# menmitsu/opticalFlowClustering

Measured on AMD Instinct MI355X. Metric: Mpixels/s dense flow+kmeans @1080p, higher is better.
Workload: dtype f32 storage, f64 accumulation; 1 GPU; BASELINE.json configs[2]: 300-frame 1080p synthetic clip, Farneback flow (0.5,3,15,3,5,1.2,0) + Lloyd k=5 over (u,v), frames sharded over 1 GPU(s); width=1920, height=1080, frames=300, pairs=299, k=5, lloyd_iters=11, flow_batch_pairs=64

## Files before the change

include/ofc.h:

```cpp
#ifndef OFC_H
#define OFC_H
#include <stddef.h>
#include <stdint.h>

#ifdef __cplusplus
extern "C" {
#endif

#define OFC_VERSION 100

enum {
    OFC_OK = 0,
    OFC_EINVAL = -1,
    OFC_ENODEV = -2,
    OFC_EHIP = -3,
    OFC_ENOMEM = -4,
    OFC_ENOTREADY = -5,
    OFC_EUNSUPPORTED = -6,
    OFC_ECOMM = -7
};

enum { OFC_U8 = 0, OFC_F32 = 1, OFC_F64 = 2 };

int ofc_version(void);
// ... 70 lines not shown
int ofc_bench_polyexp(int device, int W, int H, int n_images, int iters, int rows_per_block,
                      float *ms_per_launch);

int ofc_bgr2gray(int device, const uint8_t *bgr, int W, int H, uint8_t *gray);
int ofc_flow_to_bgr(int device, const float *flow, int W, int H, uint8_t *bgr, float *mean_mag);
int ofc_flow_to_bgr_dev(int device, const float *flow_dev, int W, int H, int n_frames,
                        uint8_t *bgr_dev, float *mean_mag_dev);
int ofc_bgr2hsv(int device, const uint8_t *bgr, int64_t npix, uint8_t *hsv);
int ofc_preprocess_rgba(int device, const uint8_t *img3, int64_t npix, int thresh, uint8_t *rgba);
int ofc_grid_cell_means(int device, const uint8_t *bgr, int W, int H, int rows, int cols,
                        uint8_t *mean_bgr, uint8_t *hsv);

int ofc_kmeans_fit(int device, const void *X, int dtype, int64_t N, int d, int k,
                   const double *init, int max_iter, double tol_rel, double *centers,
                   int32_t *labels, double *inertia, int *n_iter);
int ofc_kmeans_predict(int device, const void *X, int dtype, int64_t N, int d, int k,
                       const double *centers, int32_t *labels);
int ofc_kmeans_fit_dev(int device, const void *X_dev, int dtype, int64_t N, int d, int k,
                       const double *init, int max_iter, double tol_rel, double *centers,
                       uint8_t *labels_dev, double *inertia, int *n_iter);
int ofc_kmeans_fit_dev_stats(int device, const void *X_dev, int dtype, int64_t N, int d, int k,
                             const double *init, int max_iter, double tol_rel, const double *colsum,
                             double *centers, uint8_t *labels_dev, double *inertia, int *n_iter);
int ofc_kmeans_fit_dev_field(int device, const void *X_dev, int dtype, int64_t N, int d, int k,
                             const double *init, int max_iter, double tol_rel, const double *colsum,
                             double *centers, uint8_t *labels_dev, double *inertia, int *n_iter,
                             int W, int H, int64_t n_fields);
int64_t ofc_lloyd_field_origin(int64_t tile, int quad, int W);
int ofc_lloyd_field_origins(int64_t tile0, int64_t n_tiles, int W, int64_t *out);
void ofc_lloyd_field_shape(int *tile_w, int *tile_h, int *group_w, int *group_h);
int ofc_lloyd_prune_stats(int device, double *out6);
int ofc_bench_lloyd_sweep(int device, const float *X_dev, int64_t N, int k, const double *centers, const double *mean,
                          int what, int iters, float *ms_per_launch);
int ofc_lloyd_colstats_dev(int device, const void *X_dev, int dtype, int64_t N, int d, const double *mean,
                           int pass, double *out);
int ofc_lloyd_step_dev(int device, const void *X_dev, int dtype, int64_t N, int d, int k, const double *mean,
                       const double *centers_c, uint8_t *labels_dev, int accumulate, double *record);
int ofc_lloyd_inertia_dev(int device, const void *X_dev, int dtype, int64_t N, int d, int k, const double *mean,
                          const double *centers_c, const uint8_t *labels_dev, double *inertia);
int ofc_lloyd_farthest_dev(int device, const void *X_dev, int dtype, int64_t N, int d, int k, const double *mean,
                           const double *centers_c, const uint8_t *labels_dev, const int64_t *excl, int n_excl,
                           double *dist2, int64_t *index, double *x_c, int *label);

int ofc_kmeans_fit_w(int device, const void *X, int dtype, const void *w, int w_dtype, int64_t N, int d, int k,
                     const double *init, int max_iter, double tol_rel, double *centers, int32_t *labels,
                     double *inertia, int *n_iter);
int ofc_kmeans_fit_dev_w(int device, const void *X_dev, int dtype, const void *w_dev, int w_dtype, int64_t N, int d,
                         int k, const double *init, int max_iter, double tol_rel, const double *colsum,
                         double *centers, uint8_t *labels_dev, double *inertia, int *n_iter);
int ofc_kmeans_score(int device, const void *X, int dtype, const void *w, int w_dtype, int64_t N, int d, int k,
                     const double *centers, double *inertia);
int ofc_lloyd_step_dev_w(int device, const void *X_dev, int dtype, const void *w_dev, int w_dtype, int64_t N, int d,
                         int k, const double *mean, const double *centers_c, uint8_t *labels_dev, double *record);
int ofc_lloyd_inertia_dev_w(int device, const void *X_dev, int dtype, const void *w_dev, int w_dtype, int64_t N, int d,
                            int k, const double *mean, const double *centers_c, const uint8_t *labels_dev,
                            double *inertia);
int ofc_lloyd_farthest_dev_w(int device, const void *X_dev, int dtype, const void *w_dev, int w_dtype, int64_t N, int d,
                             int k, const double *mean, const double *centers_c, const uint8_t *labels_dev,
                             const int64_t *excl, int n_excl, double *dist2, int64_t *index, double *x_c, int *label,
                             double *weight);
int ofc_flow_weights_dev(int device, const float *flow_dev, int64_t n, int kind, float thr, float *w_dev);
int ofc_bench_lloyd_sweep_w(int device, const float *X_dev, const void *w_dev, int w_dtype, int64_t N, int k,
                            const double *centers, const double *mean, int iters, float *ms_per_launch);

int ofc_kpp_candidates(int device, const void *X, int dtype, int64_t N, int d, const double *mean,
                       const int64_t *cand, int n_cand, const double *closest, double *out_min, double *pots);
// ... 189 lines not shown
```

opticalflowclustering_amd/_lib.py:

```python
import ctypes as C
import os

import numpy as np

_HERE = os.path.dirname(os.path.abspath(__file__))
LIB_PATH = os.path.join(_HERE, "libofc.so")

OFC_OK, OFC_EINVAL, OFC_ENODEV, OFC_EHIP, OFC_ENOMEM, OFC_ENOTREADY, OFC_EUNSUPPORTED, OFC_ECOMM = \
    0, -1, -2, -3, -4, -5, -6, -7
U8, F32, F64 = 0, 1, 2
UNIQUE_ID_BYTES = 128
KPP_CHUNK = 1024
UV_HIST_SHARE = 2048
UV_HIST_MAX_GRID = 2048
BLOB_TILE_W, BLOB_TILE_H, BLOB_FIELDS = 64, 16, 12
BLOB_LINK_FIELDS, BLOB_NO_MOVE = 3, -0x7fff8000
CONSIST_OK, CONSIST_MISMATCH, CONSIST_LEAVES, CONSIST_INVALID, CONSIST_STATES = 0, 1, 2, 3, 4
CONSIST_SHARE, CONSIST_MAX_DIM = 2048, 16384
CONSIST_ALPHA_MAX, CONSIST_BETA_MAX = 65536, 1 << 62
PHOTO_SHARE, PHOTO_TAU_MAX, PHOTO_KAPPA_MAX, PHOTO_NSTAT = 2048, 65280, 1024, 5
REPAIR_ROUNDS_MAX, REPAIR_NCOUNT, REPAIR_UNFILLED = 254, 3, 255
TRAJ_RAN, TRAJ_UNTRUSTED, TRAJ_LEAVES, TRAJ_INVALID = 0, 1, 2, 3
TRAJ_THREADS, TRAJ_MAX_POINTS = 256, 1 << 28
TRAJ_ONE_LAUNCH_POINTS, TRAJ_DENSE_PAIRS = 1 << 19, 16
# ... 44 lines not shown
    "ofc_flow_push_bgr": ([_vp, _vp, _vp, C.POINTER(_f), _vp], _i),
    "ofc_flow_last_vis_dev": ([_vp, C.POINTER(_vp)], _i),
    "ofc_level_image": ([_i, _vp, _i, _i, C.POINTER(FbParams), _i, _vp, _ip, _ip], _i),
    "ofc_polyexp": ([_i, _vp, _i, _i, _i, _d, _vp], _i),
    "ofc_polyexp_u8": ([_i, _vp, _i, _i, _i, _d, _vp], _i),
    "ofc_update_matrices": ([_i, _vp, _vp, _vp, _i, _i, _vp], _i),
    "ofc_box_solve": ([_i, _vp, _i, _i, _i, _vp], _i),
    "ofc_flow_resize": ([_i, _vp, _i, _i, _i, _i, _f, _vp], _i),
    "ofc_flow_iterate": ([_i, _vp, _vp, _vp, _i, _i, _i, _i, _i, _i, _vp], _i),
    "ofc_flow_launch_geometry": ([_i, _i, _i, _i, _ip], _i),
    "ofc_flow_launch_geometry_bidir": ([_i, _i, _i, _i, _ip], _i),
    "ofc_bench_flow_bidir": ([_i, _i, _i, _i, _i, _i, C.POINTER(_f)], _i),
    "ofc_pyramid_dec": ([_i, _vp, _i, _i, _i, _i, _i, _vp, _vp, _vp, _ip], _i),
    "ofc_pyramid_dec_geometry": ([_i, _i, _i, _ip], _i),
    "ofc_bench_pyramid_dec": ([_i, _i, _i, _i, _i, _i, _i, C.POINTER(_f)], _i),
    "ofc_bench_flow_iters": ([_i, _i, _i, _i, _i, _i, C.POINTER(_f)], _i),
    "ofc_bench_polyexp": ([_i, _i, _i, _i, _i, _i, C.POINTER(_f)], _i),
    "ofc_bgr2gray": ([_i, _vp, _i, _i, _vp], _i),
    "ofc_flow_to_bgr": ([_i, _vp, _i, _i, _vp, C.POINTER(_f)], _i),
    "ofc_flow_to_bgr_dev": ([_i, _vp, _i, _i, _i, _vp, _vp], _i),
    "ofc_bgr2hsv": ([_i, _vp, _i64, _vp], _i),
    "ofc_preprocess_rgba": ([_i, _vp, _i64, _i, _vp], _i),
    "ofc_grid_cell_means": ([_i, _vp, _i, _i, _i, _i, _vp, _vp], _i),
    "ofc_kmeans_fit": ([_i, _vp, _i, _i64, _i, _i, _vp, _i, _d, _vp, _vp, C.POINTER(_d), _ip], _i),
    "ofc_kmeans_predict": ([_i, _vp, _i, _i64, _i, _i, _vp, _vp], _i),
    "ofc_kmeans_fit_dev": ([_i, _vp, _i, _i64, _i, _i, _vp, _i, _d, _vp, _vp, C.POINTER(_d), _ip], _i),
    "ofc_kmeans_fit_dev_stats": ([_i, _vp, _i, _i64, _i, _i, _vp, _i, _d, _vp, _vp, _vp, C.POINTER(_d), _ip], _i),
    "ofc_kmeans_fit_dev_field": ([_i, _vp, _i, _i64, _i, _i, _vp, _i, _d, _vp, _vp, _vp, C.POINTER(_d), _ip, _i, _i, _i64], _i),
    "ofc_lloyd_field_origin": ([_i64, _i, _i], _i64),
    "ofc_lloyd_field_origins": ([_i64, _i64, _i, _vp], _i),
    "ofc_lloyd_field_shape": ([_ip, _ip, _ip, _ip], None),
    "ofc_lloyd_prune_stats": ([_i, _vp], _i),
    "ofc_bench_lloyd_sweep": ([_i, _vp, _i64, _i, _vp, _vp, _i, _i, C.POINTER(_f)], _i),
    "ofc_lloyd_colstats_dev": ([_i, _vp, _i, _i64, _i, _vp, _i, _vp], _i),
    "ofc_lloyd_step_dev": ([_i, _vp, _i, _i64, _i, _i, _vp, _vp, _vp, _i, _vp], _i),
    "ofc_lloyd_inertia_dev": ([_i, _vp, _i, _i64, _i, _i, _vp, _vp, _vp, C.POINTER(_d)], _i),
    "ofc_lloyd_farthest_dev": ([_i, _vp, _i, _i64, _i, _i, _vp, _vp, _vp, _vp, _i, C.POINTER(_d), C.POINTER(_i64), _vp, _ip], _i),
    "ofc_kmeans_fit_w": ([_i, _vp, _i, _vp, _i, _i64, _i, _i, _vp, _i, _d, _vp, _vp, C.POINTER(_d), _ip], _i),
    "ofc_kmeans_fit_dev_w": ([_i, _vp, _i, _vp, _i, _i64, _i, _i, _vp, _i, _d, _vp, _vp, _vp, C.POINTER(_d), _ip], _i),
    "ofc_kmeans_score": ([_i, _vp, _i, _vp, _i, _i64, _i, _i, _vp, C.POINTER(_d)], _i),
    "ofc_lloyd_step_dev_w": ([_i, _vp, _i, _vp, _i, _i64, _i, _i, _vp, _vp, _vp, _vp], _i),
    "ofc_lloyd_inertia_dev_w": ([_i, _vp, _i, _vp, _i, _i64, _i, _i, _vp, _vp, _vp, C.POINTER(_d)], _i),
    "ofc_lloyd_farthest_dev_w": ([_i, _vp, _i, _vp, _i, _i64, _i, _i, _vp, _vp, _vp, _vp, _i, C.POINTER(_d), C.POINTER(_i64), _vp, _ip,
                                  C.POINTER(_d)], _i),
    "ofc_flow_weights_dev": ([_i, _vp, _i64, _i, _f, _vp], _i),
    "ofc_bench_lloyd_sweep_w": ([_i, _vp, _vp, _i, _i64, _i, _vp, _vp, _i, C.POINTER(_f)], _i),
    "ofc_kpp_candidates": ([_i, _vp, _i, _i64, _i, _vp, _vp, _i, _vp, _vp, _vp], _i),
    "ofc_kpp_seed_dev": ([_i, _vp, _i, _i64, _i, _i, _vp, _i64, _vp, _i, _vp, _vp], _i),
    "ofc_kpp_sample_dev": ([_i, _vp, _i64, _vp, _i, _vp], _i),
    "ofc_kpp_seed_dev_w": ([_i, _vp, _i, _vp, _i, _i64, _i, _i, _vp, _d, _vp, _i, _vp, _vp], _i),
    "ofc_kpp_sample_dev_w": ([_i, _vp, _i, _vp, _i64, _vp, _i, _i, _vp, _vp], _i),
    "ofc_kmeans_fit_batched": ([_i, _vp, _vp, _i, _i, _i, _vp, _i, _d, _vp, _vp, _vp, _vp], _i),
    "ofc_grid_kmeans": ([_i, _vp, _i, _i, _i, _i, _i, _vp, _i, _d, _i, _vp, _vp], _i),
    "ofc_grid_kmeans_dev": ([_i, _vp, _i, _i, _i, _i, _i, _i, _vp, _i, _d, _i, _vp, _vp], _i),
    "ofc_dist_unique_id": ([_vp], _i),
    "ofc_dist_init": ([_i, _i, _i, _vp], _i),
    "ofc_dist_allreduce_f64": ([_i, _vp, _i], _i),
    "ofc_dist_init_host": ([_i, _i, _i, _vp, _vp], _i),
    "ofc_dist_loopback": ([_i], _i),
    "ofc_dist_finalize": ([], _i),
    "ofc_stream_create": ([_i, _i, _i, C.POINTER(FbParams), _i, _i, _i, C.POINTER(_vp)], _i),
    "ofc_stream_push_gray": ([_vp, _vp, _ip], _i),
    "ofc_stream_finish": ([_vp, _vp, _i, _ip], _i),
    "ofc_stream_set_model": ([_vp, _i, _vp, _vp, _i], _i),
    "ofc_stream_finish_clusters": ([_vp, _vp, _vp, _vp, _i, _ip], _i),
    "ofc_stream_set_histogram": ([_vp, _i, _f], _i),
# ... 138 lines not shown
```

opticalflowclustering_amd/csrc/lloyd_api.cpp:

```cpp
#include "host_util.h"
#include "lloyd_common.h"

#include <algorithm>
#include <cmath>
#include <cstdlib>
#include <mutex>

namespace ofc {

static int lloyd_grid(int64_t N)
{
    return (int)std::max<int64_t>(1, std::min<int64_t>(cdiv64(N / 4, 256), N >= (200ll << 20) ? 2048 : 1024));
}

static size_t dtype_size(int dtype) { return dtype == OFC_U8 ? 1 : (dtype == OFC_F32 ? 4 : 8); }

struct LloydScratch {
    DevBuf state, partial, tot, tot_local, excl, far, labels;
    DevBuf tile_block;
    DevBuf tile_meta;
    DevBuf kpp_closest, kpp_cs, kpp_ss;
    DevBuf kpp_io;
    double prune_stats[6] = {0, 0, 0, 0, 0, 0};
    LloydStatus *status = nullptr;
// ... 142 lines not shown
    return OFC_OK;
}

static int lloyd_fit_dev(int device, const void *X, int dtype, int64_t N, int d, int k, const double *init,
                         int max_iter, double tol_rel, double *centers, uint8_t *labels_dev,
                         double *inertia, int *n_iter, const double *colsum = nullptr, const void *wdev = nullptr,
                         int w_dtype = OFC_F32, int field_w = 0, int field_h = 0, int64_t n_fields = 0)
{
    OFC_REQUIRE(X && init && centers, "null pointer");
    OFC_REQUIRE(dtype >= OFC_U8 && dtype <= OFC_F64, "bad dtype %d", dtype);
    OFC_REQUIRE(!wdev || w_dtype == OFC_F32 || w_dtype == OFC_F64, "bad weight dtype %d (OFC_F32 or OFC_F64)", w_dtype);
    OFC_REQUIRE(d >= 1 && k >= 1 && max_iter >= 1 && N >= 0, "bad shape");
    if (d > LLOYD_DMAX || k > LLOYD_KMAX) {
        set_error("k=%d, d=%d outside the kernels' range (k <= %d, d <= %d)", k, d, LLOYD_KMAX, LLOYD_DMAX);
        return OFC_EUNSUPPORTED;
    }
    OFC_TRY(ensure_device(device));
    const int kmax = lloyd_kmax(k);
    const int NV = lloyd_record_len(kmax, d);
    LloydScratch &sc = scratch_for(device);
    std::lock_guard<std::mutex> lock(sc.mu);
    OFC_TRY(sc.init());
    hipStream_t s = sc.stream;
    const int nblocks = lloyd_grid(N);
    if (!labels_dev) {
        OFC_TRY(reserve(sc.labels, (size_t)std::max<int64_t>(N, 1)));
        labels_dev = sc.labels.as<uint8_t>();
    }
    LloydState *st = sc.state.as<LloydState>();
    OFC_HIP(hipMemsetAsync(st, 0, sizeof(LloydState), s));
    double *tot = sc.tot.as<double>();

    double hbuf[LLOYD_DMAX + 1], mean_h[LLOYD_DMAX];
    if (colsum) {
        OFC_HIP(hipMemcpyAsync(tot, colsum, sizeof(double) * d, hipMemcpyHostToDevice, s));
    } else {
        OFC_TRY(launch_lloyd_colstats(X, dtype, N, d, st->mean, 0, sc.partial.as<double>(), nblocks, s));
        OFC_TRY(launch_reduce_records(sc.partial.as<double>(), nblocks, d, tot, s));
    }
    double nloc = (double)N;
    OFC_HIP(hipMemcpyAsync(tot + d, &nloc, sizeof(double), hipMemcpyHostToDevice, s));
    OFC_TRY(dist_allreduce_f64(tot, d + 1, DIST_SUM, s));
    OFC_HIP(hipMemcpyAsync(hbuf, tot, sizeof(double) * (d + 1), hipMemcpyDeviceToHost, s));
    OFC_HIP(hipStreamSynchronize(s));
    const double Ng = hbuf[d];
    if (Ng < (double)k) {
        set_error("n_samples=%.0f should be >= n_clusters=%d.", Ng, k);
        return OFC_EINVAL;
    }
    for (int f = 0; f < d; f++) mean_h[f] = hbuf[f] / Ng;
    OFC_HIP(hipMemcpyAsync(st->mean, mean_h, sizeof(double) * d, hipMemcpyHostToDevice, s));

    double c0[LLOYD_KMAX * LLOYD_DMAX];
    for (int j = 0; j < k * d; j++) c0[j] = init[j] - mean_h[j % d];
    OFC_HIP(hipMemcpyAsync(st->centers, c0, sizeof(double) * k * d, hipMemcpyHostToDevice, s));
    const int prune = wdev ? LLOYD_PRUNE_OFF : prune_policy_for(dtype, N, d, k);
    const bool field = prune && field_w > 0 && field_geometry_ok(field_w, field_h, n_fields);
    LloydFieldBufs tb = {};
    if (prune) OFC_TRY(sc.tile_bufs(N, field ? field_w : 0, tb));
    auto tiles_launch = [&](uint8_t *lab, int what, const double *meta) -> int {
        if (field) return launch_lloyd_tiles_field((const float *)X, N, k, st, tb, lab, sc.partial.as<double>(), nblocks, what, meta, s);
        return launch_lloyd_tiles((const float *)X, N, k, st, tb.box, tb.tsum, tb.tsq, lab, sc.partial.as<double>(), nblocks, what,
                                  meta, s);
    };
    for (double &v : sc.prune_stats) v = 0;
    OFC_TRY(launch_lloyd_set_centers(st, k, d, s, prune));
    bool strict = false, labelled = false, stop = false;
    int tiles_next = LLOYD_TILES_FULL;
    const bool trace = getenv("OFC_LLOYD_TRACE") != nullptr;
    int it = 0;
    const int *halt = &st->halt;
    double *tot_local = dist_has_comm() ? sc.tot_local.as<double>() : tot;
    int window = 4;
    while (it < max_iter && !stop) {
        const int nwin = std::min(window, max_iter - it);
        window = std::min(2 * window, LLOYD_WINDOW);
        for (int w = 0; w < nwin; w++) sc.status[w].valid = 0;
// ... 132 lines not shown
    std::lock_guard<std::mutex> lock(sc.mu);
    OFC_TRY(sc.init());
    hipStream_t s = sc.stream;
    const int nblocks = lloyd_grid(N);
    LloydFieldBufs tb = {};
    OFC_TRY(sc.tile_bufs(N, 0, tb));
    OFC_TRY(reserve(sc.labels, (size_t)N));
    LloydState *st = sc.state.as<LloydState>();
    OFC_HIP(hipMemsetAsync(st, 0, sizeof(LloydState), s));
    double c0[LLOYD_KMAX * LLOYD_DMAX];
    for (int j = 0; j < k * 2; j++) c0[j] = centers[j] - mean[j % 2];
    OFC_HIP(hipMemcpyAsync(st->mean, mean, sizeof(double) * 2, hipMemcpyHostToDevice, s));
    OFC_HIP(hipMemcpyAsync(st->centers, c0, sizeof(double) * k * 2, hipMemcpyHostToDevice, s));
    OFC_TRY(launch_lloyd_set_centers(st, k, 2, s, LLOYD_PRUNE_ALWAYS));
    double *partial = sc.partial.as<double>();
    const float *X = X_dev;
    auto launch = [&]() -> int {
        switch (what) {
        case 0: return launch_lloyd_assign(X, OFC_F32, N, 2, k, st, sc.labels.as<uint8_t>(), partial, nblocks, 3, 0, s);
        case 1: case 5: return launch_lloyd_tiles(X, N, k, st, tb.box, tb.tsum, tb.tsq, nullptr, partial, nblocks, LLOYD_WHAT_SWEEP, nullptr, s);
        case 2: return launch_lloyd_tiles(X, N, k, st, tb.box, tb.tsum, tb.tsq, nullptr, partial, nblocks, LLOYD_WHAT_META, nullptr, s);
        case 3: return launch_lloyd_assign(X, OFC_F32, N, 2, k, st, sc.labels.as<uint8_t>(), partial, nblocks, 2, 0, s);
        default: return launch_lloyd_tiles(X, N, k, st, tb.box, tb.tsum, tb.tsq, sc.labels.as<uint8_t>(), partial, nblocks, LLOYD_WHAT_FINAL, nullptr, s);
        }
    };
    if (what == 1 || what == 4 || what == 5) {
        OFC_TRY(launch_lloyd_tiles(X, N, k, st, tb.box, tb.tsum, tb.tsq, nullptr, partial, nblocks, LLOYD_WHAT_META, nullptr, s));
        const int mode = what == 5 ? LLOYD_TILES_FULL : LLOYD_TILES_PRUNED;
        OFC_HIP(hipMemcpyAsync(&st->prune_mode, &mode, sizeof(int), hipMemcpyHostToDevice, s));
    }
    return time_launches(s, iters, launch, ms_per_launch);
}

int ofc_lloyd_prune_stats(int device, double *out6)
{
    OFC_REQUIRE(out6, "null pointer");
    OFC_TRY(ensure_device(device));
    LloydScratch &sc = scratch_for(device);
    std::lock_guard<std::mutex> lock(sc.mu);
    for (int i = 0; i < 6; i++) out6[i] = sc.prune_stats[i];
    return OFC_OK;
}

int ofc_kmeans_fit_dev_stats(int device, const void *X_dev, int dtype, int64_t N, int d, int k, const double *init,
                             int max_iter, double tol_rel, const double *colsum, double *centers, uint8_t *labels_dev,
                             double *inertia, int *n_iter)
{
    return lloyd_fit_dev(device, X_dev, dtype, N, d, k, init, max_iter, tol_rel, centers, labels_dev, inertia, n_iter, colsum);
}

int ofc_kmeans_fit_dev_field(int device, const void *X_dev, int dtype, int64_t N, int d, int k, const double *init,
                             int max_iter, double tol_rel, const double *colsum, double *centers, uint8_t *labels_dev,
                             double *inertia, int *n_iter, int W, int H, int64_t n_fields)
{
    OFC_REQUIRE(dtype == OFC_F32 && d == 2, "a stack of (u,v) fields is float32 with d = 2 (got dtype %d, d = %d)", dtype, d);
    OFC_REQUIRE(W >= 1 && H >= 1 && n_fields >= 1 && N / W / H == n_fields && n_fields * W * H == N,
                "N=%lld is not %lld fields of %d x %d", (long long)N, (long long)n_fields, W, H);
    return lloyd_fit_dev(device, X_dev, dtype, N, d, k, init, max_iter, tol_rel, centers, labels_dev, inertia, n_iter, colsum,
                         nullptr, OFC_F32, W, H, n_fields);
}

int64_t ofc_lloyd_field_origin(int64_t tile, int quad, int W)
{
    if (tile < 0 || quad < 0 || quad > 15 || W < FIELD_GW || W % FIELD_GW) return -1;
    return field_quad_origin(tile, quad, W);
}
// ... 758 lines not shown
```

opticalflowclustering_amd/csrc/lloyd_field.h:

```cpp
#pragma once
#include <cstdint>

#ifndef __host__
#define __host__
#define __device__
#endif

namespace ofc {

#ifndef OFC_FIELD_TW
#define OFC_FIELD_TW 16
#endif
constexpr int FIELD_TW = OFC_FIELD_TW, FIELD_TH = 64 / FIELD_TW;
constexpr int FIELD_GW = 64, FIELD_GH = 8;
constexpr int FIELD_GTX = FIELD_GW / FIELD_TW, FIELD_GTY = FIELD_GH / FIELD_TH;
constexpr int FIELD_QPR = FIELD_TW / 4;
static_assert(FIELD_TW * FIELD_TH == 64 && FIELD_GTX * FIELD_GTY == 8 && FIELD_QPR >= 1 && FIELD_TH <= FIELD_GH, "tile shape");

__host__ __device__ inline bool field_geometry_ok(int64_t W, int64_t H, int64_t n_fields)
{
    return W > 0 && H > 0 && n_fields > 0 && W % FIELD_GW == 0 && H % FIELD_GH == 0 && W <= (1 << 24) &&
           n_fields * H <= (int64_t)0x7fffffff / W * 4;
}
__host__ __device__ inline int64_t field_group_origin(int64_t g, int W)
{
    const int64_t gx_n = W / FIELD_GW, band = g / gx_n;
    return band * FIELD_GH * W + (g - band * gx_n) * FIELD_GW;
}
__host__ __device__ inline int field_tile_offset(int ti, int W)
{
    return (ti / FIELD_GTX) * FIELD_TH * W + (ti % FIELD_GTX) * FIELD_TW;
}
__host__ __device__ inline int field_quad_offset(int r16, int W)
{
    return (r16 / FIELD_QPR) * W + (r16 % FIELD_QPR) * 4;
}
__host__ __device__ inline int64_t field_quad_origin(int64_t t, int r16, int W)
{
    return field_group_origin(t >> 3, W) + field_tile_offset((int)(t & 7), W) + field_quad_offset(r16, W);
}

}
```

opticalflowclustering_amd/csrc/lloyd_tiles.hip:

```cpp
#include "lloyd_common.h"

#include <algorithm>

namespace ofc {

typedef float v4f __attribute__((ext_vector_type(4)));
typedef double v2d __attribute__((ext_vector_type(2)));

template <int N> __device__ __forceinline__ int row_ror(int v)
{
    return __builtin_amdgcn_update_dpp(0, v, 0x120 + N, 0xf, 0xf, false);
}
template <int N> __device__ __forceinline__ float row_ror(float v) { return __int_as_float(row_ror<N>(__float_as_int(v))); }
template <int N> __device__ __forceinline__ double row_ror(double v)
{
    return __hiloint2double(row_ror<N>(__double2hiint(v)), row_ror<N>(__double2loint(v)));
}
__device__ __forceinline__ float row_min(float v)
{
    v = fminf(v, row_ror<8>(v)); v = fminf(v, row_ror<4>(v)); v = fminf(v, row_ror<2>(v)); return fminf(v, row_ror<1>(v));
}
__device__ __forceinline__ float row_max(float v)
{
    v = fmaxf(v, row_ror<8>(v)); v = fmaxf(v, row_ror<4>(v)); v = fmaxf(v, row_ror<2>(v)); return fmaxf(v, row_ror<1>(v));
// ... 396 lines not shown
{
    __shared__ double s_cen[KMAX][4];
    __shared__ unsigned s_red[4][2];
    TileCtx<KMAX> cx;
    cx.load(st, s_cen);
    const int tid = threadIdx.x, lane = tid & 63, wave = tid >> 6, row = lane >> 4, r16 = lane & 15;
    const int64_t NT = N >> 6, NS = NT >> 2;
    const int64_t nw = (int64_t)gridDim.x * 4, w = (int64_t)blockIdx.x * 4 + wave;
    const int64_t stride = NS > 64 * nw ? 64 : (NS > nw ? NS / nw : 1);
    unsigned n_tested = 0, n_pure = 0;
    for (int64_t s = w * stride; s < NS; s += nw * stride) {
        const int64_t t = s * 4 + row;
        const v4f *p = reinterpret_cast<const v4f *>(X + field_quad_origin(t, r16, W) * 2);
        const v4f a = p[0], b = p[1];
        const float lu = row_min(fminf(fminf(a.x, a.z), fminf(b.x, b.z)));
        const float lv = row_min(fminf(fminf(a.y, a.w), fminf(b.y, b.w)));
        const float hu = row_max(fmaxf(fmaxf(a.x, a.z), fmaxf(b.x, b.z)));
        const float hv = row_max(fmaxf(fmaxf(a.y, a.w), fmaxf(b.y, b.w)));
        const int tl = cx.box_label((double)lu - cx.m[0], (double)lv - cx.m[1], (double)hu - cx.m[0], (double)hv - cx.m[1]);
        if (r16 == 0) {
            n_tested += 1u;
            n_pure += (tl >= 0);
        }
    }
    for (int off = 32; off >= 1; off >>= 1) {
        n_tested += __shfl_down(n_tested, off, 64);
        n_pure += __shfl_down(n_pure, off, 64);
    }
    if (lane == 0) { s_red[wave][0] = n_tested; s_red[wave][1] = n_pure; }
    __syncthreads();
    if (tid < 2) partial[(size_t)blockIdx.x * 2 + tid] = (double)(s_red[0][tid] + s_red[1][tid] + s_red[2][tid] + s_red[3][tid]);
}

__global__ __launch_bounds__(256) void k_tile_meta_field(const float *__restrict__ X, int64_t N, int W,
                                                         const LloydState *__restrict__ st, v4f *__restrict__ box,
                                                         v2d *__restrict__ tsum, double *__restrict__ tsq,
                                                         v4f *__restrict__ gbox, v2d *__restrict__ gsum,
                                                         double *__restrict__ gsq, double *__restrict__ partial)
{
    __shared__ double s_red[4][2];
    const int tid = threadIdx.x, lane = tid & 63, wave = tid >> 6, row = lane >> 4, r16 = lane & 15;
    if (st->prune_policy == LLOYD_PRUNE_OFF) {
        if (tid < 2) partial[(size_t)blockIdx.x * 2 + tid] = 0.0;
        return;
    }
    const double m0 = st->mean[0], m1 = st->mean[1];
    const int NGr = (int)(N >> 9);
    const int g0 = blockIdx.x * 4 + wave, gs = gridDim.x * 4;
    const int off[2] = {field_tile_offset(row, W) + field_quad_offset(r16, W), field_tile_offset(4 + row, W) + field_quad_offset(r16, W)};
    double sq0 = 0, sq1 = 0;
    auto fetch = [&](int g, v4f (&q)[4]) {
        if (g < NGr) {
            const float *o = X + field_group_origin(g, W) * 2;
#pragma unroll
            for (int h = 0; h < 2; h++) {
                const v4f *p = reinterpret_cast<const v4f *>(o + (int64_t)off[h] * 2);
                q[2 * h] = __builtin_nontemporal_load(p);
                q[2 * h + 1] = __builtin_nontemporal_load(p + 1);
            }
        }
    };
    v4f nq[4] = {{0, 0, 0, 0}, {0, 0, 0, 0}, {0, 0, 0, 0}, {0, 0, 0, 0}};
    fetch(g0, nq);
    for (int g = g0; g < NGr; g += gs) {
        v4f q[4];
#pragma unroll
        for (int i = 0; i < 4; i++) q[i] = nq[i];
        fetch(g + gs, nq);
        float lu[2], lv[2], hu[2], hv[2];
        double su[2], sv[2], sc[2];
        bool bad = false;
#pragma unroll
        for (int h = 0; h < 2; h++) {
            const v4f a = q[2 * h], b = q[2 * h + 1];
            const double x00 = (double)a.x - m0, x01 = (double)a.y - m1, x10 = (double)a.z - m0, x11 = (double)a.w - m1;
            const double x20 = (double)b.x - m0, x21 = (double)b.y - m1, x30 = (double)b.z - m0, x31 = (double)b.w - m1;
            sq0 += x00 * x00; sq0 += x10 * x10; sq0 += x20 * x20; sq0 += x30 * x30;
            sq1 += x01 * x01; sq1 += x11 * x11; sq1 += x21 * x21; sq1 += x31 * x31;
            lu[h] = row_min(fminf(fminf(a.x, a.z), fminf(b.x, b.z)));
            lv[h] = row_min(fminf(fminf(a.y, a.w), fminf(b.y, b.w)));
            hu[h] = row_max(fmaxf(fmaxf(a.x, a.z), fmaxf(b.x, b.z)));
            hv[h] = row_max(fmaxf(fmaxf(a.y, a.w), fmaxf(b.y, b.w)));
            su[h] = row_sum((x00 + x10) + (x20 + x30));
            sv[h] = row_sum((x01 + x11) + (x21 + x31));
            const double mu = su[h] * 0.015625, mv = sv[h] * 0.015625;
            double s = (x00 - mu) * (x00 - mu) + (x01 - mv) * (x01 - mv);
            s += (x10 - mu) * (x10 - mu) + (x11 - mv) * (x11 - mv);
            s += (x20 - mu) * (x20 - mu) + (x21 - mv) * (x21 - mv);
            s += (x30 - mu) * (x30 - mu) + (x31 - mv) * (x31 - mv);
            sc[h] = row_sum(s);
            const bool tbad = !(su[h] == su[h] && sv[h] == sv[h]);
            bad = bad || tbad;
            if (r16 == 0) {
                const int64_t t = (int64_t)g * 8 + h * 4 + row;
                v4f bx = {lu[h], lv[h], hu[h], hv[h]};
                if (tbad) bx = v4f{__builtin_inff(), __builtin_inff(), -__builtin_inff(), -__builtin_inff()};
                box[t] = bx;
                tsum[t] = v2d{su[h], sv[h]};
                tsq[t] = sc[h];
            }
        }
        const double gu = rows_sum(su[0]) + rows_sum(su[1]), gv = rows_sum(sv[0]) + rows_sum(sv[1]);
        const double mgu = gu * 0.001953125, mgv = gv * 0.001953125;
        double term = 0;
#pragma unroll
        for (int h = 0; h < 2; h++) {
            const double du = su[h] * 0.015625 - mgu, dv = sv[h] * 0.015625 - mgv;
            term += sc[h] + 64.0 * (du * du + dv * dv);
        }
        const double gsc = rows_sum(term);
        const float glu = rows_min(fminf(lu[0], lu[1])), glv = rows_min(fminf(lv[0], lv[1]));
        const float ghu = rows_max(fmaxf(hu[0], hu[1])), ghv = rows_max(fmaxf(hv[0], hv[1]));
        const bool gbad = __any(bad) || !(gu == gu && gv == gv);
        if (lane == 0) {
            v4f bx = {glu, glv, ghu, ghv};
            if (gbad) bx = v4f{__builtin_inff(), __builtin_inff(), -__builtin_inff(), -__builtin_inff()};
            gbox[g] = bx;
            gsum[g] = v2d{gu, gv};
            gsq[g] = gsc;
        }
    }
    for (int off2 = 32; off2 >= 1; off2 >>= 1) {
        sq0 += __shfl_down(sq0, off2, 64);
        sq1 += __shfl_down(sq1, off2, 64);
    }
    if (lane == 0) { s_red[wave][0] = sq0; s_red[wave][1] = sq1; }
    __syncthreads();
    if (tid < 2) partial[(size_t)blockIdx.x * 2 + tid] = ((s_red[0][tid] + s_red[1][tid]) + s_red[2][tid]) + s_red[3][tid];
}

template <int KMAX, int WHAT>
__global__ __launch_bounds__(256) void k_lloyd_tiles_field(const float *__restrict__ X, int64_t N, int W,
                                                           const LloydState *__restrict__ st, const v4f *__restrict__ box,
                                                           const v2d *__restrict__ tsum, const double *__restrict__ tsq,
                                                           const v4f *__restrict__ gbox, const v2d *__restrict__ gsum,
                                                           const double *__restrict__ gsq, uint8_t *__restrict__ labels,
                                                           double *__restrict__ partial, const double *__restrict__ meta)
{
    constexpr int D = 2, k = KMAX;
    constexpr int NV = KMAX * D + KMAX + LLOYD_REC_EXTRA;
    constexpr bool FINAL = WHAT == TILES_FINAL, ACCUM = !FINAL;
    if (ACCUM && st->halt) return;
    const int mode = ACCUM ? st->prune_mode : LLOYD_TILES_PRUNED;
    const bool own_sq = ACCUM && meta && st->prune_policy == LLOYD_PRUNE_OFF;
    double sq0 = 0, sq1 = 0;
    extern __shared__ __align__(16) unsigned char smem[];
    double *sacc = reinterpret_cast<double *>(smem);
    unsigned *scnt = reinterpret_cast<unsigned *>(sacc + (size_t)k * D * 256);
    __shared__ unsigned s_tiles[4][2];
    __shared__ double s_cen[KMAX][4];
    const int tid = threadIdx.x, lane = tid & 63, wave = tid >> 6, row = lane >> 4, r16 = lane & 15;
    if (ACCUM) {
        for (int i = 0; i < k * D; i++) sacc[i * 256 + tid] = 0.0;
        for (int j = 0; j < k; j++) scnt[j * 256 + tid] = 0u;
    }
    TileCtx<KMAX> cx;
    cx.load(st, s_cen);
    double inert = 0;
    unsigned n_tested = 0, n_pure = 0;
    auto accumulate = [&](int l, double x0, double x1, unsigned n) {
        sacc[(l * D) * 256 + tid] += x0;
        sacc[(l * D + 1) * 256 + tid] += x1;
// ... 295 lines not shown
```

opticalflowclustering_amd/stages.py:

```python
import ctypes as C

import numpy as np

from ._lib import FbParams, check, load, ptr


def level_image(gray, k, params=None, device=0):
    gray = np.ascontiguousarray(gray, np.uint8)
    H, W = gray.shape
    p = params or FbParams()
    out = np.empty((H, W), np.float32)
    w, h = C.c_int(), C.c_int()
    check(load().ofc_level_image(device, ptr(gray), W, H, C.byref(p), k, ptr(out), C.byref(w), C.byref(h)))
    return out.reshape(-1)[: w.value * h.value].reshape(h.value, w.value).copy()


def pyramid_dec(frames, levels, fused=True, device=0):
    frames = np.ascontiguousarray(frames, np.uint8)
    n, H, W = frames.shape
    outs = [np.empty((n, int(np.rint(H * 0.5 ** k)), int(np.rint(W * 0.5 ** k))), np.float32) for k in range(1, levels + 1)]
    ptrs = [ptr(o) for o in outs] + [None] * (3 - levels)
    nf = C.c_int(-1)
    check(load().ofc_pyramid_dec(device, ptr(frames), n, W, H, levels, int(bool(fused)), *ptrs, C.byref(nf)))
    return outs, nf.value
# ... 68 lines not shown

def bench_flow_bidir(W, H, n_frames, reps, what, device=0):
    ms = C.c_float()
    check(load().ofc_bench_flow_bidir(device, W, H, n_frames, reps, what, C.byref(ms)))
    return ms.value


def bench_flow_iters(W, H, n_pairs, reps, mode, device=0):
    ms = C.c_float()
    check(load().ofc_bench_flow_iters(device, W, H, n_pairs, reps, mode, C.byref(ms)))
    return ms.value


def bench_pyramid_dec(W, H, n_images, levels=3, fused=True, iters=20, device=0):
    ms = C.c_float()
    check(load().ofc_bench_pyramid_dec(device, W, H, n_images, levels, int(bool(fused)), iters, C.byref(ms)))
    return ms.value


def bench_polyexp(W, H, n_images, iters, rows_per_block=0, device=0):
    ms = C.c_float()
    check(load().ofc_bench_polyexp(device, W, H, n_images, iters, rows_per_block, C.byref(ms)))
    return ms.value


def bench_lloyd_sweep(X_ptr, N, centers, mean, what, iters=10, device=0):
    cen = np.ascontiguousarray(centers, np.float64)
    mean = np.ascontiguousarray(mean, np.float64)
    ms = C.c_float()
    check(load().ofc_bench_lloyd_sweep(device, C.c_void_p(X_ptr), N, len(cen), ptr(cen), ptr(mean), what, iters, C.byref(ms)))
    return ms.value


def bench_lloyd_sweep_w(X_ptr, w_ptr, w_dtype, N, centers, mean, iters=10, device=0):
    cen = np.ascontiguousarray(centers, np.float64)
    mean = np.ascontiguousarray(mean, np.float64)
    ms = C.c_float()
    check(load().ofc_bench_lloyd_sweep_w(device, C.c_void_p(X_ptr), C.c_void_p(w_ptr), w_dtype, N, len(cen), ptr(cen), ptr(mean),
                                         iters, C.byref(ms)))
    return ms.value


def bench_uv_hist(flow_ptr, n, bins=1024, range=32.0, iters=10, device=0):
    ms = C.c_float()
    check(load().ofc_bench_uv_hist(device, C.c_void_p(flow_ptr), n, bins, range, iters, C.byref(ms)))
    return ms.value


def flow_weights_dev(flow_ptr, n, kind, thr, w_ptr, device=0):
    kinds = {"magnitude": 0, "moving": 1}
    if kind not in kinds:
        raise ValueError(f"weight kind should be 'magnitude' or 'moving', got {kind!r}")
    check(load().ofc_flow_weights_dev(device, C.c_void_p(flow_ptr), n, kinds[kind], float(thr), C.c_void_p(w_ptr)))
```

Before: 19370 Mpixels/s.

## Deepen tile-meta prefetch, coalesce per-tile stores, skip colsum round-trip

The tile-metadata kernel now prefetches two groups ahead with clamped unconditional loads, and uses asm barriers to keep the loads in flight across the compute. Per-tile box/sum/sq results are gathered via shuffles so that 8 lanes write contiguous stores, instead of scattered writes from lane r16==0. Row reductions use unmasked DPP rotates and the wave index is made uniform. The host fit skips the device upload/allreduce/sync of colsum when there is no communicator. The change also adds a benchmark entry point for the meta kernel. The clamped loads add redundant memory traffic on the last iterations, and the asm constraints could inhibit other compiler optimizations.

Result: no change. 19260 Mpixels/s (-0.6%).

```diff
diff --git a/include/ofc.h b/include/ofc.h
--- a/include/ofc.h
+++ b/include/ofc.h
@@ -126,6 +126,9 @@
 int ofc_lloyd_prune_stats(int device, double *out6);
 int ofc_bench_lloyd_sweep(int device, const float *X_dev, int64_t N, int k, const double *centers, const double *mean,
                           int what, int iters, float *ms_per_launch);
+int ofc_lloyd_field_meta(int device, const float *X_dev, int W, int H, int64_t n_fields, const double *mean, void *box,
+                         void *tsum, void *tsq, void *gbox, void *gsum, void *gsq, double *colsq, int *grid, int iters,
+                         float *ms_per_launch);
 int ofc_lloyd_colstats_dev(int device, const void *X_dev, int dtype, int64_t N, int d, const double *mean,
                            int pass, double *out);
 int ofc_lloyd_step_dev(int device, const void *X_dev, int dtype, int64_t N, int d, int k, const double *mean,
diff --git a/opticalflowclustering_amd/_lib.py b/opticalflowclustering_amd/_lib.py
--- a/opticalflowclustering_amd/_lib.py
+++ b/opticalflowclustering_amd/_lib.py
@@ -100,6 +100,7 @@
     "ofc_lloyd_field_shape": ([_ip, _ip, _ip, _ip], None),
     "ofc_lloyd_prune_stats": ([_i, _vp], _i),
     "ofc_bench_lloyd_sweep": ([_i, _vp, _i64, _i, _vp, _vp, _i, _i, C.POINTER(_f)], _i),
+    "ofc_lloyd_field_meta": ([_i, _vp, _i, _i, _i64, _vp, _vp, _vp, _vp, _vp, _vp, _vp, _vp, _ip, _i, C.POINTER(_f)], _i),
     "ofc_lloyd_colstats_dev": ([_i, _vp, _i, _i64, _i, _vp, _i, _vp], _i),
     "ofc_lloyd_step_dev": ([_i, _vp, _i, _i64, _i, _i, _vp, _vp, _vp, _i, _vp], _i),
     "ofc_lloyd_inertia_dev": ([_i, _vp, _i, _i64, _i, _i, _vp, _vp, _vp, C.POINTER(_d)], _i),
diff --git a/opticalflowclustering_amd/csrc/lloyd_api.cpp b/opticalflowclustering_amd/csrc/lloyd_api.cpp
--- a/opticalflowclustering_amd/csrc/lloyd_api.cpp
+++ b/opticalflowclustering_amd/csrc/lloyd_api.cpp
@@ -198,17 +198,22 @@
     double *tot = sc.tot.as<double>();
 
     double hbuf[LLOYD_DMAX + 1], mean_h[LLOYD_DMAX];
-    if (colsum) {
-        OFC_HIP(hipMemcpyAsync(tot, colsum, sizeof(double) * d, hipMemcpyHostToDevice, s));
+    if (colsum && !dist_has_comm()) {
+        for (int f = 0; f < d; f++) hbuf[f] = colsum[f];
+        hbuf[d] = (double)N;
     } else {
-        OFC_TRY(launch_lloyd_colstats(X, dtype, N, d, st->mean, 0, sc.partial.as<double>(), nblocks, s));
-        OFC_TRY(launch_reduce_records(sc.partial.as<double>(), nblocks, d, tot, s));
-    }
-    double nloc = (double)N;
-    OFC_HIP(hipMemcpyAsync(tot + d, &nloc, sizeof(double), hipMemcpyHostToDevice, s));
-    OFC_TRY(dist_allreduce_f64(tot, d + 1, DIST_SUM, s));
-    OFC_HIP(hipMemcpyAsync(hbuf, tot, sizeof(double) * (d + 1), hipMemcpyDeviceToHost, s));
-    OFC_HIP(hipStreamSynchronize(s));
+        if (colsum) {
+            OFC_HIP(hipMemcpyAsync(tot, colsum, sizeof(double) * d, hipMemcpyHostToDevice, s));
+        } else {
+            OFC_TRY(launch_lloyd_colstats(X, dtype, N, d, st->mean, 0, sc.partial.as<double>(), nblocks, s));
+            OFC_TRY(launch_reduce_records(sc.partial.as<double>(), nblocks, d, tot, s));
+        }
+        double nloc = (double)N;
+        OFC_HIP(hipMemcpyAsync(tot + d, &nloc, sizeof(double), hipMemcpyHostToDevice, s));
+        OFC_TRY(dist_allreduce_f64(tot, d + 1, DIST_SUM, s));
+        OFC_HIP(hipMemcpyAsync(hbuf, tot, sizeof(double) * (d + 1), hipMemcpyDeviceToHost, s));
+        OFC_HIP(hipStreamSynchronize(s));
+    }
     const double Ng = hbuf[d];
     if (Ng < (double)k) {
         set_error("n_samples=%.0f should be >= n_clusters=%d.", Ng, k);
@@ -407,6 +412,41 @@
     return time_launches(s, iters, launch, ms_per_launch);
 }
 
+int ofc_lloyd_field_meta(int device, const float *X_dev, int W, int H, int64_t n_fields, const double *mean, void *box,
+                         void *tsum, void *tsq, void *gbox, void *gsum, void *gsq, double *colsq, int *grid, int iters,
+                         float *ms_per_launch)
+{
+    OFC_REQUIRE(X_dev && mean && iters >= 0 && (iters == 0 || ms_per_launch), "bad arguments");
+    OFC_REQUIRE(field_geometry_ok(W, H, n_fields), "%lld fields of %d x %d cannot be cut into 2-D tiles", (long long)n_fields, W, H);
+    OFC_TRY(ensure_device(device));
+    LloydScratch &sc = scratch_for(device);
+    std::lock_guard<std::mutex> lock(sc.mu);
+    OFC_TRY(sc.init());
+    hipStream_t s = sc.stream;
+    const int64_t N = n_fields * W * H;
+    const int nblocks = lloyd_grid(N);
+    LloydFieldBufs tb = {};
+    OFC_TRY(sc.tile_bufs(N, W, tb));
+    LloydState *st = sc.state.as<LloydState>();
+    OFC_HIP(hipMemsetAsync(st, 0, sizeof(LloydState), s));
+    OFC_HIP(hipMemcpyAsync(st->mean, mean, sizeof(double) * 2, hipMemcpyHostToDevice, s));
+    OFC_TRY(launch_lloyd_set_centers(st, 1, 2, s, LLOYD_PRUNE_ALWAYS));
+    double *partial = sc.partial.as<double>();
+    auto launch = [&]() -> int { return launch_lloyd_tiles_field(X_dev, N, 1, st, tb, nullptr, partial, nblocks, LLOYD_WHAT_META, nullptr, s); };
+    OFC_TRY(launch());
+    OFC_TRY(launch_reduce_records(partial, nblocks, 2, sc.tile_meta.as<double>(), s));
+    const size_t nt = (size_t)(N >> 6), ng = nt >> 3;
+    const struct { void *dst; const void *src; size_t bytes; } out[] = {
+        {box, tb.box, nt * 16}, {tsum, tb.tsum, nt * 16}, {tsq, tb.tsq, nt * 8}, {gbox, tb.gbox, ng * 16},
+        {gsum, tb.gsum, ng * 16}, {gsq, tb.gsq, ng * 8}, {colsq, sc.tile_meta.p, sizeof(double) * 2}};
+    for (const auto &o : out)
+        if (o.dst) OFC_HIP(hipMemcpyAsync(o.dst, o.src, o.bytes, hipMemcpyDeviceToHost, s));
+    OFC_HIP(hipStreamSynchronize(s));
+    if (grid) *grid = nblocks;
+    if (iters > 0) OFC_TRY(time_launches(s, iters, launch, ms_per_launch));
+    return OFC_OK;
+}
+
 int ofc_lloyd_prune_stats(int device, double *out6)
 {
     OFC_REQUIRE(out6, "null pointer");
diff --git a/opticalflowclustering_amd/csrc/lloyd_field.h b/opticalflowclustering_amd/csrc/lloyd_field.h
--- a/opticalflowclustering_amd/csrc/lloyd_field.h
+++ b/opticalflowclustering_amd/csrc/lloyd_field.h
@@ -27,6 +27,11 @@
     const int64_t gx_n = W / FIELD_GW, band = g / gx_n;
     return band * FIELD_GH * W + (g - band * gx_n) * FIELD_GW;
 }
+__host__ __device__ inline int64_t field_group_origin_u32(unsigned g, int W)
+{
+    const unsigned gx_n = (unsigned)W / FIELD_GW, band = g / gx_n;
+    return (int64_t)band * FIELD_GH * W + (int64_t)(g - band * gx_n) * FIELD_GW;
+}
 __host__ __device__ inline int field_tile_offset(int ti, int W)
 {
     return (ti / FIELD_GTX) * FIELD_TH * W + (ti % FIELD_GTX) * FIELD_TW;
diff --git a/opticalflowclustering_amd/csrc/lloyd_tiles.hip b/opticalflowclustering_amd/csrc/lloyd_tiles.hip
--- a/opticalflowclustering_amd/csrc/lloyd_tiles.hip
+++ b/opticalflowclustering_amd/csrc/lloyd_tiles.hip
@@ -452,6 +452,26 @@
     if (tid < 2) partial[(size_t)blockIdx.x * 2 + tid] = (double)(s_red[0][tid] + s_red[1][tid] + s_red[2][tid] + s_red[3][tid]);
 }
 
+template <int N> __device__ __forceinline__ int row_ror_u(int v) { return __builtin_amdgcn_mov_dpp(v, 0x120 + N, 0xf, 0xf, false); }
+template <int N> __device__ __forceinline__ float row_ror_u(float v) { return __int_as_float(row_ror_u<N>(__float_as_int(v))); }
+template <int N> __device__ __forceinline__ double row_ror_u(double v)
+{
+    return __hiloint2double(row_ror_u<N>(__double2hiint(v)), row_ror_u<N>(__double2loint(v)));
+}
+__device__ __forceinline__ float row_min_u(float v)
+{
+    v = fminf(v, row_ror_u<8>(v)); v = fminf(v, row_ror_u<4>(v)); v = fminf(v, row_ror_u<2>(v)); return fminf(v, row_ror_u<1>(v));
+}
+__device__ __forceinline__ float row_max_u(float v)
+{
+    v = fmaxf(v, row_ror_u<8>(v)); v = fmaxf(v, row_ror_u<4>(v)); v = fmaxf(v, row_ror_u<2>(v)); return fmaxf(v, row_ror_u<1>(v));
+}
+__device__ __forceinline__ double row_sum_u(double v)
+{
+    v += row_ror_u<8>(v); v += row_ror_u<4>(v); v += row_ror_u<2>(v); return v + row_ror_u<1>(v);
+}
+
+#define OFC_META_PTRS "s"(X), "s"(box), "s"(tsum), "s"(tsq), "s"(gbox), "s"(gsum), "s"(gsq)
 __global__ __launch_bounds__(256) void k_tile_meta_field(const float *__restrict__ X, int64_t N, int W,
                                                          const LloydState *__restrict__ st, v4f *__restrict__ box,
                                                          v2d *__restrict__ tsum, double *__restrict__ tsq,
@@ -459,7 +479,8 @@
                                                          double *__restrict__ gsq, double *__restrict__ partial)
 {
     __shared__ double s_red[4][2];
-    const int tid = threadIdx.x, lane = tid & 63, wave = tid >> 6, row = lane >> 4, r16 = lane & 15;
+    const int tid = threadIdx.x, lane = tid & 63, row = lane >> 4, r16 = lane & 15;
+    const int wave = __builtin_amdgcn_readfirstlane(tid >> 6);
     if (st->prune_policy == LLOYD_PRUNE_OFF) {
         if (tid < 2) partial[(size_t)blockIdx.x * 2 + tid] = 0.0;
         return;
@@ -468,28 +489,27 @@
     const int NGr = (int)(N >> 9);
     const int g0 = blockIdx.x * 4 + wave, gs = gridDim.x * 4;
     const int off[2] = {field_tile_offset(row, W) + field_quad_offset(r16, W), field_tile_offset(4 + row, W) + field_quad_offset(r16, W)};
+    const int hsel = (r16 >> 2) & 1, src = (lane & 3) * 16 + (lane & 4);
+    const v4f poison = {__builtin_inff(), __builtin_inff(), -__builtin_inff(), -__builtin_inff()};
     double sq0 = 0, sq1 = 0;
     auto fetch = [&](int g, v4f (&q)[4]) {
-        if (g < NGr) {
-            const float *o = X + field_group_origin(g, W) * 2;
-#pragma unroll
-            for (int h = 0; h < 2; h++) {
-                const v4f *p = reinterpret_cast<const v4f *>(o + (int64_t)off[h] * 2);
-                q[2 * h] = __builtin_nontemporal_load(p);
-                q[2 * h + 1] = __builtin_nontemporal_load(p + 1);
-            }
-        }
+        const float *o = X + field_group_origin_u32((unsigned)(g < NGr ? g : NGr - 1), W) * 2;
+#pragma unroll
+        for (int h = 0; h < 2; h++) {
+            const v4f *p = reinterpret_cast<const v4f *>(o + (int64_t)off[h] * 2);
+            q[2 * h] = __builtin_nontemporal_load(p);
+            q[2 * h + 1] = __builtin_nontemporal_load(p + 1);
+        }
+        asm volatile("" : : OFC_META_PTRS : "memory");
     };
-    v4f nq[4] = {{0, 0, 0, 0}, {0, 0, 0, 0}, {0, 0, 0, 0}, {0, 0, 0, 0}};
-    fetch(g0, nq);
+    v4f q[4], nq[4];
+    fetch(g0, q);
+    fetch(g0 + gs, nq);
+    asm volatile("" : "+v"(q[0]), "+v"(q[1]), "+v"(q[2]), "+v"(q[3]) : OFC_META_PTRS : "memory");
     for (int g = g0; g < NGr; g += gs) {
-        v4f q[4];
-#pragma unroll
-        for (int i = 0; i < 4; i++) q[i] = nq[i];
-        fetch(g + gs, nq);
         float lu[2], lv[2], hu[2], hv[2];
         double su[2], sv[2], sc[2];
-        bool bad = false;
+        bool tbad[2];
 #pragma unroll
         for (int h = 0; h < 2; h++) {
             const v4f a = q[2 * h], b = q[2 * h + 1];
@@ -497,29 +517,21 @@
             const double x20 = (double)b.x - m0, x21 = (double)b.y - m1, x30 = (double)b.z - m0, x31 = (double)b.w - m1;
             sq0 += x00 * x00; sq0 += x10 * x10; sq0 += x20 * x20; sq0 += x30 * x30;
             sq1 += x01 * x01; sq1 += x11 * x11; sq1 += x21 * x21; sq1 += x31 * x31;
-            lu[h] = row_min(fminf(fminf(a.x, a.z), fminf(b.x, b.z)));
-            lv[h] = row_min(fminf(fminf(a.y, a.w), fminf(b.y, b.w)));
-            hu[h] = row_max(fmaxf(fmaxf(a.x, a.z), fmaxf(b.x, b.z)));
-            hv[h] = row_max(fmaxf(fmaxf(a.y, a.w), fmaxf(b.y, b.w)));
-            su[h] = row_sum((x00 + x10) + (x20 + x30));
-            sv[h] = row_sum((x01 + x11) + (x21 + x31));
+            lu[h] = row_min_u(fminf(fminf(a.x, a.z), fminf(b.x, b.z)));
+            lv[h] = row_min_u(fminf(fminf(a.y, a.w), fminf(b.y, b.w)));
+            hu[h] = row_max_u(fmaxf(fmaxf(a.x, a.z), fmaxf(b.x, b.z)));
+            hv[h] = row_max_u(fmaxf(fmaxf(a.y, a.w), fmaxf(b.y, b.w)));
+            su[h] = row_sum_u((x00 + x10) + (x20 + x30));
+            sv[h] = row_sum_u((x01 + x11) + (x21 + x31));
             const double mu = su[h] * 0.015625, mv = sv[h] * 0.015625;
             double s = (x00 - mu) * (x00 - mu) + (x01 - mv) * (x01 - mv);
             s += (x10 - mu) * (x10 - mu) + (x11 - mv) * (x11 - mv);
             s += (x20 - mu) * (x20 - mu) + (x21 - mv) * (x21 - mv);
             s += (x30 - mu) * (x30 - mu) + (x31 - mv) * (x31 - mv);
-            sc[h] = row_sum(s);
-            const bool tbad = !(su[h] == su[h] && sv[h] == sv[h]);
-            bad = bad || tbad;
-            if (r16 == 0) {
-                const int64_t t = (int64_t)g * 8 + h * 4 + row;
-                v4f bx = {lu[h], lv[h], hu[h], hv[h]};
-                if (tbad) bx = v4f{__builtin_inff(), __builtin_inff(), -__builtin_inff(), -__builtin_inff()};
-                box[t] = bx;
-                tsum[t] = v2d{su[h], sv[h]};
-                tsq[t] = sc[h];
-            }
-        }
+            sc[h] = row_sum_u(s);
+            tbad[h] = !(su[h] == su[h] && sv[h] == sv[h]);
+        }
+        const bool bad = tbad[0] || tbad[1];
         const double gu = rows_sum(su[0]) + rows_sum(su[1]), gv = rows_sum(sv[0]) + rows_sum(sv[1]);
         const double mgu = gu * 0.001953125, mgv = gv * 0.001953125;
         double term = 0;
@@ -532,13 +544,28 @@
         const float glu = rows_min(fminf(lu[0], lu[1])), glv = rows_min(fminf(lv[0], lv[1]));
         const float ghu = rows_max(fmaxf(hu[0], hu[1])), ghv = rows_max(fmaxf(hv[0], hv[1]));
         const bool gbad = __any(bad) || !(gu == gu && gv == gv);
+        const v4f b0 = tbad[0] ? poison : v4f{lu[0], lv[0], hu[0], hv[0]}, b1 = tbad[1] ? poison : v4f{lu[1], lv[1], hu[1], hv[1]};
+        const v4f bw = hsel ? b1 : b0;
+        const v4f bx = {__shfl(bw.x, src, 64), __shfl(bw.y, src, 64), __shfl(bw.z, src, 64), __shfl(bw.w, src, 64)};
+        const v2d ts = {__shfl(hsel ? su[1] : su[0], src, 64), __shfl(hsel ? sv[1] : sv[0], src, 64)};
+        const double tq = __shfl(hsel ? sc[1] : sc[0], src, 64);
+        __builtin_amdgcn_sched_barrier(0);
+        asm volatile("" : "+v"(nq[0]), "+v"(nq[1]), "+v"(nq[2]), "+v"(nq[3]) : OFC_META_PTRS : "memory");
+        if (lane < 8) {
+            const int64_t t = (int64_t)g * 8 + lane;
+            box[t] = bx;
+            tsum[t] = ts;
+            tsq[t] = tq;
+        }
         if (lane == 0) {
-            v4f bx = {glu, glv, ghu, ghv};
-            if (gbad) bx = v4f{__builtin_inff(), __builtin_inff(), -__builtin_inff(), -__builtin_inff()};
-            gbox[g] = bx;
+            gbox[g] = gbad ? poison : v4f{glu, glv, ghu, ghv};
             gsum[g] = v2d{gu, gv};
             gsq[g] = gsc;
         }
+        asm volatile("" : : OFC_META_PTRS : "memory");
+#pragma unroll
+        for (int i = 0; i < 4; i++) q[i] = nq[i];
+        fetch(g + 2 * gs, nq);
     }
     for (int off2 = 32; off2 >= 1; off2 >>= 1) {
         sq0 += __shfl_down(sq0, off2, 64);
@@ -548,6 +575,7 @@
     __syncthreads();
     if (tid < 2) partial[(size_t)blockIdx.x * 2 + tid] = ((s_red[0][tid] + s_red[1][tid]) + s_red[2][tid]) + s_red[3][tid];
 }
+#undef OFC_META_PTRS
 
 template <int KMAX, int WHAT>
 __global__ __launch_bounds__(256) void k_lloyd_tiles_field(const float *__restrict__ X, int64_t N, int W,
diff --git a/opticalflowclustering_amd/stages.py b/opticalflowclustering_amd/stages.py
--- a/opticalflowclustering_amd/stages.py
+++ b/opticalflowclustering_amd/stages.py
@@ -124,6 +124,25 @@
     return ms.value
 
 
+def lloyd_field_meta(X_ptr, W, H, n_fields, mean, copy=True, iters=0, device=0):
+    n = int(n_fields) * W * H
+    nt, ng = n // 64, n // 512
+    mean = np.ascontiguousarray(mean, np.float64)
+    out = {}
+    if copy:
+        out = dict(box=np.empty((nt, 4), np.float32), tsum=np.empty((nt, 2), np.float64), tsq=np.empty(nt, np.float64),
+                   gbox=np.empty((ng, 4), np.float32), gsum=np.empty((ng, 2), np.float64), gsq=np.empty(ng, np.float64))
+    colsq = np.empty(2, np.float64)
+    grid, ms = C.c_int(), C.c_float()
+    args = [ptr(out[k]) if copy else None for k in ("box", "tsum", "tsq", "gbox", "gsum", "gsq")]
+    check(load().ofc_lloyd_field_meta(device, C.c_void_p(X_ptr), W, H, int(n_fields), ptr(mean), *args, ptr(colsq),
+                                      C.byref(grid), iters, C.byref(ms)))
+    out.update(colsq=colsq, grid=grid.value)
+    if iters > 0:
+        out["ms"] = ms.value
+    return out
+
+
 def bench_lloyd_sweep_w(X_ptr, w_ptr, w_dtype, N, centers, mean, iters=10, device=0):
     cen = np.ascontiguousarray(centers, np.float64)
     mean = np.ascontiguousarray(mean, np.float64)
```
